# fhgyuanshen/HybridGL

Measured on AMD Instinct MI355X. Metric: images/sec (whole node), higher is better.
Workload: dtype f32 via fp16x3 split MFMA (fp32 accumulate)

## Files before the change

### hybridgl_amd/_lib.py

```python
import ctypes as C
import os

_HERE = os.path.dirname(os.path.abspath(__file__))
LIB_PATH = os.path.join(_HERE, "libhybridgl.so")

c_float_p = C.POINTER(C.c_float)
c_u8_p = C.POINTER(C.c_uint8)
c_i32_p = C.POINTER(C.c_int32)
c_i64_p = C.POINTER(C.c_int64)


class HybridGLError(RuntimeError):
    pass


class HglSentence(C.Structure):
    _fields_ = [("sentence_row", C.c_int), ("noun_phrase_row", C.c_int), ("other_row0", C.c_int), ("n_other", C.c_int),
                ("dirflag", C.c_int), ("relaword", C.c_int), ("has_other_nouns", C.c_int), ("black", C.c_float),
                ("imgattn", C.c_void_p), ("target", C.c_void_p)]


class HglGroupRef(C.Structure):
    _fields_ = [("hybrid", C.c_void_p), ("text", C.c_void_p), ("T", C.c_int), ("boxes", C.c_void_p), ("masks", C.c_void_p),
                ("N", C.c_int), ("H", C.c_int), ("W", C.c_int), ("sentences", C.POINTER(HglSentence)), ("S", C.c_int),
# ... 141 lines not shown
                                  _VP, _VP, _SZ, _VP]),
    "hgl_sam_relpos_tables_workspace_bytes": (_SZ, [_I, _I, _I, _I]),
    "hgl_sam_relpos_tables": (_I, [_VP, _VP, _VP, _I, _I, _I, _I, _I, _I, _VP, _VP, _VP, _VP, _VP, _SZ, _VP]),
    "hgl_sam_dense_pe": (_I, [C.POINTER(HglSamDecoderW), _VP, _VP, _VP]),
    "hgl_sam_decode_workspace_bytes": (_SZ, [C.POINTER(HglSamDecoderW), _I]),
    "hgl_sam_decode_points": (_I, [C.POINTER(HglSamDecoderW), _VP, _VP, _I, _VP, _VP, _VP, _SZ, _VP]),
    "hgl_sam_decode_points_gated": (_I, [C.POINTER(HglSamDecoderW), _VP, _VP, _I, C.c_float, _VP, _VP, _VP, _SZ, _VP]),
    "hgl_sam_decode_multi_workspace_bytes": (_SZ, [C.POINTER(HglSamDecoderW), _I, _I]),
    "hgl_sam_decode_points_multi": (_I, [C.POINTER(HglSamDecoderW), _VP, _VP, _I, _I, _VP, _VP, _VP, _SZ, _VP]),
    "hgl_sam_decode_points_multi_gated": (_I, [C.POINTER(HglSamDecoderW), _VP, _VP, _I, _I, C.c_float, _VP, _VP, _VP, _SZ, _VP]),
    "hgl_sam_decode_prompts": (_I, [C.POINTER(HglSamDecoderW), _VP, _VP, _VP, _I, _VP, _I, _I, _VP, _VP, _VP, _SZ, _VP]),
    "hgl_sam_embed_masks": (_I, [C.POINTER(HglSamDecoderW), _VP, _I, _VP, _VP]),
    "hgl_sam_decoder_fusion": (_I, [_I]),
    "hgl_attention_presplit": (_I, [_I]),
    "hgl_attention_presplit_f32": (_I, [_VP, _I, _I, _I, _I, _I, _VP, _I, C.c_float, _I, _VP, _I, _I, _VP, C.c_size_t, _VP]),
    "hgl_sam_postprocess_workspace_bytes": (_SZ, [_I]),
    "hgl_sam_postprocess": (_I, [_VP, _VP, _I, _I, _I, _I, _I, _I, _I, _I, _F, _F, _F, _F, _VP, _VP, _VP, _VP, _VP,
                                 _VP, _SZ, _VP]),
    "hgl_nms": (_I, [_VP, _VP, _VP, _I, _F, _VP, _VP, _VP]),
    "hgl_nms_segments": (_I, [_VP, _VP, _VP, _VP, _I, _I, _F, _VP, _VP, _VP]),
    "hgl_nms_large_workspace_bytes": (_SZ, [_I]),
    "hgl_nms_large": (_I, [_VP, _VP, _VP, _I, _F, _VP, _VP, _VP, _SZ, _VP]),
    "hgl_box_near_crop_edge": (_I, [_VP, _I, C.POINTER(C.c_int32), C.POINTER(C.c_int32), _F, _VP, _VP]),
    "hgl_remove_small_regions_workspace_bytes": (_SZ, [_I, _I, _I]),
    "hgl_remove_small_regions": (_I, [_VP, _I, _I, _I, _I, _I, _VP, _VP, _VP, _SZ, _VP]),
    "hgl_remove_small_regions_boxes": (_I, [_VP, _I, _I, _I, _I, _I, _VP, _VP, _VP, _VP, _SZ, _VP]),
    "hgl_mask_boxes": (_I, [_VP, _I, _I, _I, _VP, _VP]),
    "hgl_gather_masks": (_I, [_VP, _VP, _VP, _I, _LL, _VP, _VP]),
    "hgl_gen_dir_mask": (_I, [_I, _I, _I, _VP, _VP]),
    "hgl_relation_boxes": (_I, [_VP, _VP, _VP, _VP, _I, _I, _VP, _VP]),
# ... 74 lines not shown
```

### hybridgl_amd/csrc/attention_ps.hip

```cpp
#include "hgl_common.h"
#include "attn_tile.h"
#include <stdlib.h>
#include <mutex>
#include <type_traits>

namespace {

typedef __attribute__((address_space(3))) void lds_void_t;

constexpr int PS_CHUNK = 32;

enum { PS_PLAIN = 0, PS_WIN14 = 1, PS_RELT = 2 };

struct PsArgs {
  const _Float16 *hi, *lo;
  int ld, qcol, kcol, vcol;
  long long sb;
  int B, H, S;
  float* out;
  _Float16 *out_hi, *out_lo;
  int ldo;
  long long sob;
  float scale;
  int mask_kind;
  const uint8_t* keep;
  int keep_b0, keep_n;
  const float *rel_h, *rel_w;
  int kh, kw;
  const _Float16 *tabh_hi, *tabh_lo, *tabw_hi, *tabw_lo;
  int nqb;
  int dbg;
};
#ifdef HGL_DIAG
#define PS_DBG(a) ((a).dbg)
#else
#define PS_DBG(a) 0
#endif

__device__ __forceinline__ void ps_glds16(const void* sbase, unsigned voff, unsigned lds_addr) {
  unsigned keep;
  asm volatile("s_mov_b32 %0, m0\n\ts_mov_b32 m0, %3\n\ts_nop 0\n\tglobal_load_lds_dwordx4 %1, %2\n\ts_mov_b32 m0, %0"
               : "=&s"(keep)
               : "v"(voff), "s"(sbase), "s"(lds_addr)
               : "memory");
// ... 293 lines not shown
      const unsigned krow = min((unsigned)(ci * PS_CHUNK) + v_row[j], (unsigned)(a.S - 1));
      ps_glds16(kv_base, krow * ldb + v_col[j], sbase + (unsigned)(wave + 4 * j) * 1024u);
    }
  };
  const int nchunk = (a.S + PS_CHUNK - 1) / PS_CHUNK;
  if constexpr (MODE == PS_WIN14) {
    for (int i = wave; i < PSP_EBYTES / 1024; i += 4) ps_glds16(etab, (unsigned)(i * 1024 + lane * 16), lds0 + G::E_OFF + (unsigned)i * 1024u);
  }
  const int tr_off = attn_tr_off<VP>(lane, h);
  const int k_off = r * KP + 8 * h;
  int e_off[2];
#pragma unroll
  for (int c = 0; c < 2; ++c) e_off[c] = r * 64 + (((2 * c + h) ^ ((r >> 2) & 3)) * 16);

  const unsigned nunits = (unsigned)(a.B * a.H) * (unsigned)a.nqb;
  for (unsigned L = blockIdx.x; L < nunits; L += gridDim.x) {
  int item, bx;
  {
    const unsigned nqb = (unsigned)a.nqb;
    if ((a.B & 7) == 0) {
      int be, rem;
      attn_xcd_item(L, (unsigned)a.H * nqb, be, rem);
      item = (int)((unsigned)be * (unsigned)a.H + (unsigned)rem / nqb);
      bx = (int)((unsigned)rem % nqb);
    } else {
      item = (int)(L / nqb);
      bx = (int)(L % nqb);
    }
  }
  const int b = item / a.H, hh = item - b * a.H;
  kv_base = (const char*)a.hi + ((long long)b * a.sb * (long long)a.ld + a.kcol + hh * HD) * 2;
  if (L != blockIdx.x) __syncthreads();
  if (!(PS_DBG(a) & 4)) {
  issue_k(0);
  issue_v(0);
// ... 342 lines not shown
            const auto s0 = __builtin_amdgcn_permlane32_swap(x[0], y[0], false, false);
            const auto s1 = __builtin_amdgcn_permlane32_swap(x[1], y[1], false, false);
            return u32x4s{(unsigned)s0[0], (unsigned)s1[0], (unsigned)s0[1], (unsigned)s1[1]};
          };
          const u32x4s vh = pair16(hi0, hi1), vl = pair16(lo0, lo1);
          if (qvalid[qt]) {
            const long long off = orow + d * 32 + 8 * g + 8 * h;
            *(u32x4s*)(a.out_hi + off) = vh;
            *(u32x4s*)(a.out_lo + off) = vl;
          }
        }
      }
  }
  }
  }
}

const unsigned char* psp_etab() {
  static const unsigned char* tab[64] = {nullptr};
  static std::mutex mu;
  std::lock_guard<std::mutex> lk(mu);
  int dev = 0;
  if (hipGetDevice(&dev) != hipSuccess || dev < 0 || dev >= 64) dev = 0;
  if (!tab[dev]) {
    static unsigned short host[PS_EROWS * 32];
    for (int row = 0; row < PS_EROWS; ++row)
      for (int j = 0; j < 32; ++j) {
        const int ih = row / 14, iw = 14 + row % 14;
        const int chunk = j >> 3, phys = chunk ^ ((row >> 2) & 3);
        host[row * 32 + phys * 8 + (j & 7)] = (j == ih || j == iw) ? 0x3c00 : 0;
// ... 51 lines not shown
#ifdef HGL_PS_STAMPS
extern "C" int hgl_debug_ps_stamps(unsigned long long* out, int n, int block, int wave) {
  (void)hipMemcpyFromSymbol(out, HIP_SYMBOL(g_ps_stamps), sizeof(unsigned long long) * (n < 1024 ? n : 1024));
  unsigned long long z[1024] = {0};
  (void)hipMemcpyToSymbol(HIP_SYMBOL(g_ps_stamps), z, sizeof(z));
  int sel[2] = {block, wave};
  (void)hipMemcpyToSymbol(HIP_SYMBOL(g_ps_stamp_sel), sel, sizeof(sel));
  return 0;
}
#endif

extern "C" int hgl_attention_presplit(int on) {
  const int prev = attn_ps_flag();
  if (on >= 0) g_attn_ps = on != 0;
  return prev;
}

HglAttnRoute hgl_attention_route_planes(const HglAttn& d) {
  const int S = d.Sq, hd = d.hd;
  if (!(attn_ps_flag() != 0 && hgl_split_layout() && hgl_split_terms() == 3) || d.Sk != S) return HGL_ATTN_NONE;
  if (!(hd == 80 || hd == 64) || d.mask_kind == HGL_MASK_CAUSAL || d.B <= 0 || d.H <= 0 || S <= 0) return HGL_ATTN_NONE;
  const long long plane_delta = (const char*)d.qkv_lo - (const char*)d.qkv_hi;
  const long long span = (long long)S * d.ld * 2 + (long long)d.ld * 2;
  if (plane_delta < 0 || plane_delta + span >= (1ll << 32)) return HGL_ATTN_NONE;
  static const int clip_kernel = HGL_DIAG_SWITCH("HGL_ATTN_PS_CLIP", 1);
  const int rel_kh = d.rel_h ? d.kh : 0, rel_kw = d.rel_h ? d.kw : 0;
  if (d.tab_h || d.tab_w) {
    const void* t[4];
    return hd == 80 && S == 196 && d.mask_kind == HGL_MASK_NONE && !rel_kh && hgl_attention_rel_tables(d.tab_h, d.tab_w, t)
               ? HGL_ATTN_PS_WIN
// ... 16 lines not shown
  HGL_REQUIRE((d.ld & 7) == 0 && (d.qcol & 7) == 0 && (d.kcol & 7) == 0 && (d.vcol & 7) == 0 && (d.ldo & 3) == 0 && (d.sob & 3) == 0 &&
                  (((uintptr_t)d.qkv_hi | (uintptr_t)d.qkv_lo | (uintptr_t)d.out | (uintptr_t)d.out_hi | (uintptr_t)d.out_lo) & 15) == 0,
              "attention_ps: operands must be 16-byte aligned");
  HGL_REQUIRE(d.mask_kind != HGL_MASK_CLS_KEEP || d.keep, "attention_ps: HGL_MASK_CLS_KEEP needs keep bytes");
  HGL_REQUIRE(d.vcol >= d.kcol, "attention_ps: the V columns must not lie before the K columns (32-bit offsets from the K base)");
  HGL_REQUIRE((d.rel_h == nullptr) == (d.rel_w == nullptr) && (d.tab_h == nullptr) == (d.tab_w == nullptr), "attention_ps: rel-pos operands go in pairs");
  PsArgs a;
  a.hi = (const _Float16*)d.qkv_hi; a.lo = (const _Float16*)d.qkv_lo;
  a.ld = d.ld; a.qcol = d.qcol; a.kcol = d.kcol; a.vcol = d.vcol; a.sb = d.sb;
  a.B = d.B; a.H = d.H; a.S = S;
  a.out = d.out; a.out_hi = (_Float16*)d.out_hi; a.out_lo = (_Float16*)d.out_lo; a.ldo = d.ldo; a.sob = d.sob;
  a.scale = d.scale; a.mask_kind = d.mask_kind; a.keep = d.keep; a.keep_b0 = d.keep_b0; a.keep_n = d.keep_n > 0 ? d.keep_n : d.B;
  a.rel_h = d.rel_h; a.rel_w = d.rel_w; a.kh = d.kh; a.kw = d.kw;
  a.tabh_hi = a.tabh_lo = a.tabw_hi = a.tabw_lo = nullptr;
  a.nqb = 1;
  a.dbg = HGL_DIAG_SWITCH("HGL_ATTN_PS_DBG", 0);
  if (route == HGL_ATTN_PS_WIN) {
    const void* t[4];
    (void)hgl_attention_rel_tables(d.tab_h, d.tab_w, t);
    a.tabh_hi = (const _Float16*)t[0]; a.tabh_lo = (const _Float16*)t[1];
    a.tabw_hi = (const _Float16*)t[2]; a.tabw_lo = (const _Float16*)t[3];
    a.nqb = 2;
  } else if (route != HGL_ATTN_PS_CLIP) {
    a.nqb = (S + 127) / 128;
  }
  HglProfScope prof(HGL_PROF_ATTN, 4.0 * d.B * d.H * (double)S * S * d.hd, 0.0, st);
  switch (route) {
    case HGL_ATTN_PS_WIN: return psp_launch<80, PS_WIN14>(a, st);
    case HGL_ATTN_PS_RELT: return d.hd == 80 ? psp_launch<80, PS_RELT>(a, st) : psp_launch<64, PS_RELT>(a, st);
    case HGL_ATTN_PS_PLAIN: return d.hd == 80 ? psp_launch<80, PS_PLAIN>(a, st) : psp_launch<64, PS_PLAIN>(a, st);
    default: return ps_launch<64, PS_PLAIN, 2>(a, st);
  }
}

extern "C" int hgl_attention_presplit_f32(const float* qkv, int ld, int B, int H, int S, int hd, float* out, int ldo, float scale,
                                          int mask_kind, const uint8_t* keep, int keep_b0, int keep_n, void* scratch,
                                          size_t scratch_bytes, void* stream) {
// ... 5 lines not shown
  hipStream_t st = (hipStream_t)stream;
  uint16_t* hi = (uint16_t*)scratch;
  uint16_t* lo = hi + n;
  HGL_TRY(hgl_launch_split_f16(qkv, 1.0f, hi, lo, (long long)n, st));
  HglAttn d = hgl_attn_packed_planes(hi, lo, B, H, S, hd);
  d.ld = ld, d.scale = scale;
  d.out = out, d.ldo = ldo, d.sob = (long long)S * ldo;
  d.mask_kind = mask_kind, d.keep = keep, d.keep_b0 = keep_b0, d.keep_n = keep_n;
  const int prev = hgl_attention_presplit(1);
  const bool served = hgl_attention_route(d) != HGL_ATTN_NONE;
  const int rc = served ? hgl_launch_attention(d, st) : HGL_OK;
  hgl_attention_presplit(prev);
  HGL_REQUIRE(served, "attention_presplit: shape not served (B %d, H %d, S %d, hd %d, mask %d)", B, H, S, hd, mask_kind);
  return rc;
}
```

### hybridgl_amd/csrc/hgl_common.h

```cpp
#pragma once
#include <hip/hip_runtime.h>
#include <stdint.h>
#include <stddef.h>
#include <math.h>
#include <atomic>
#include <type_traits>
#include "../../include/hybridgl.h"

typedef float f32x16 __attribute__((ext_vector_type(16)));
typedef float f32x4 __attribute__((ext_vector_type(4)));

#ifdef __HIPCC__
static __device__ __attribute__((unused)) unsigned int hgl_tu_split_overflow;
__device__ __forceinline__ void hgl_split_hi_lo(float x, _Float16& hi, _Float16& lo) {
  asm volatile("" : "+v"(x));
  hi = (_Float16)x;
  lo = (_Float16)(x - (float)hi);
}
__device__ __forceinline__ void hgl_split_hi_lo(float x, _Float16& hi, _Float16& lo, float& amax) {
  asm volatile("" : "+v"(x));
  amax = fmaxf(amax, fabsf(x));
  hi = (_Float16)x;
  lo = (_Float16)(x - (float)hi);
}
// ... 171 lines not shown
  int ldq = 0, ldk = 0, ldv = 0;
  long long sqb = 0, skb = 0, svb = 0;
  const void *qkv_hi = nullptr, *qkv_lo = nullptr;
  int ld = 0, qcol = 0, kcol = 0, vcol = 0;
  long long sb = 0;
  float* out = nullptr;
  void *out_hi = nullptr, *out_lo = nullptr;
  int ldo = 0;
  long long sob = 0;
  int mask_kind = HGL_MASK_NONE;
  const uint8_t* keep = nullptr;
  int keep_b0 = 0, keep_n = 0;
  const float *rel_h = nullptr, *rel_w = nullptr;
  int kh = 0, kw = 0;
  const float *tab_h = nullptr, *tab_w = nullptr;
  float* part = nullptr;
  size_t part_bytes = 0;
  int kv_group = 1;
};
inline HglAttn hgl_attn_packed(const float* qkv, int B, int H, int S, int hd) {
  const int D = H * hd;
  HglAttn d;
  d.B = B, d.H = H, d.Sq = S, d.Sk = S, d.hd = hd, d.scale = 1.0f / sqrtf((float)hd);
  d.q = qkv, d.k = qkv + D, d.v = qkv + 2 * D;
  d.ldq = d.ldk = d.ldv = 3 * D;
  d.sqb = d.skb = d.svb = (long long)S * 3 * D;
  d.ldo = D, d.sob = (long long)S * D;
  return d;
}
inline HglAttn hgl_attn_packed_planes(const void* hi, const void* lo, int B, int H, int S, int hd) {
// ... 13 lines not shown
  HGL_ATTN_SMALLK,
  HGL_ATTN_F32,
  HGL_ATTN_PINGPONG,
  HGL_ATTN_REL14,
  HGL_ATTN_DUAL,
  HGL_ATTN_WIDE,
  HGL_ATTN_TILE,
  HGL_ATTN_PS_WIN,
  HGL_ATTN_PS_RELT,
  HGL_ATTN_PS_CLIP,
  HGL_ATTN_PS_PLAIN
};
HglAttnRoute hgl_attention_route(const HglAttn& d);
int hgl_launch_attention(const HglAttn& d, hipStream_t st);
size_t hgl_attention_fewq_part_bytes(int B, int Sk);
bool hgl_attention_rel_tables(const float* tab_h, const float* tab_w, const void* t[4]);
HglAttnRoute hgl_attention_route_planes(const HglAttn& d);
int hgl_launch_attention_planes(const HglAttn& d, HglAttnRoute route, hipStream_t st);

int hgl_launch_im2col_patch(const float* img, int N, int res, int patch, float* cols, hipStream_t st);
int hgl_launch_im2col_patch_split(const float* img, int N, int res, int patch, void* hi, void* lo, hipStream_t st);
int hgl_launch_assemble_lnpre(const float* tok, const float* cls, const float* pos, const float* lw,
                              const float* lb, float* x, int B, int S, int D, hipStream_t st);
int hgl_launch_mask_resize(const uint8_t* masks, int N, int Hm, int Wm, int g, float* pm,
                           uint8_t* keep, hipStream_t st);
int hgl_launch_mix(float* out, const float* a, float ca, const float* b, float cb, const float* pm,
                   int N, int S, int D, hipStream_t st);
int hgl_launch_gather_rows(const float* x, long long row_stride, int rows, int D, float* y,
                           hipStream_t st);
int hgl_launch_add_inplace(float* y, const float* x, long long n, hipStream_t st);
// ... 40 lines not shown
                             float* rel, hipStream_t st);
int hgl_launch_relpos_direct(const float* qkv, int ldq, int B, int heads, int S, int size, int hd,
                             const float* Rh, const float* Rw, float* rel_h, float* rel_w, hipStream_t st);
int hgl_launch_relpos_split(const void* q_hi, const void* q_lo, int ldq, int B, int heads, int S, int size, int hd,
                            const float* Rh, const float* Rw, float* rel_h, float* rel_w, hipStream_t st);
int hgl_launch_im2col3x3(const float* in, int g, int C, float* cols, hipStream_t st);
int hgl_launch_add_rows_bcast(const float* a, long long a_bstride, const float* pe, long long rows_elems,
                              int B, float* out, hipStream_t st);
int hgl_launch_pe(const float* coords01, const float* G, int n, int F, int mode, const float* pos_embed,
                  const float* not_a_point, float* out, hipStream_t st);
int hgl_launch_build_tokens(const float* iou_tok, const float* mask_tok, const float* sparse, int P, int C, int T,
                            float* tokens, hipStream_t st);
int hgl_launch_mask_downscaling(const float* in, int P, int g, const float* c1w, const float* c1b, const float* n1w, const float* n1b,
                                const float* c2w, const float* c2b, const float* n2w, const float* n2b, const float* c3w,
                                const float* c3b, float* out, hipStream_t st);
int hgl_launch_win_maps(int g, int ws, int nw, int nb, int* pad_of, int* tok_of, int* pad_list, int* pad_count, hipStream_t st);
int hgl_launch_fill_rows(float* dst, int ld, const int* rows, const int* nrows, int max_rows, const float* v, int N,
                         hipStream_t st);
int hgl_launch_fill_rows_split(void* hi, void* lo, int ld, const int* rows, const int* nrows, int max_rows, const float* v,
                               int N, hipStream_t st);
int hgl_launch_ln_gelu64(float* x, const float* w, const float* b, long long rows, float eps, void* hi, void* lo,
                         hipStream_t st);
int hgl_launch_ln256_pe_split(float* x, const float* w, const float* b, const float* pe, int pe_rows, long long rows,
                              float eps, int write_f32, void* kh, void* kl, void* ph, void* pl, hipStream_t st);
int hgl_launch_hyper_logits(const float* u2, const float* hyper, int P, int g, int row0, float* low_res, hipStream_t st);
int hgl_launch_pe_labeled(const float* coords01, const int32_t* labels, const float* G, int n, int F, const float* not_a_point,
                          const float* const* point_embed, float* out, hipStream_t st);
int hgl_launch_t2i_fold_q(const float* q1, const float* Wk, float scale, float* Qk, int P, hipStream_t st);
int hgl_t2i_key_ranges(int P, int HW);
size_t hgl_t2i_part_bytes(int P, int HW);
int hgl_launch_t2i_raw_attn(const void* Qh, const void* Ql, const float* bias, const void* Kh, const void* Kl, int P, int HW,
// ... 36 lines not shown
```

### hybridgl_amd/csrc/sam_api.hip

```cpp
#include "hgl_common.h"
#include <stdlib.h>
#include <math.h>

namespace {

struct EncPlan {
  float *img, *cols, *X, *H, *Hw, *QKV, *O, *P, *F, *Th, *Tw, *relh, *relw, *neckA, *neckB, *cols3;
  int *pad_of, *tok_of, *pad_list, *pad_count;
  int n_pad_max;
  int nb;
};

bool carve_enc(HglArena& ar, const HglSamEncoderW* w, int nb, EncPlan& p) {
  const int D = w->embed_dim, S = w->img_size, g = S / w->patch, C = w->out_chans;
  const size_t T = (size_t)nb * g * g;
  size_t Tw_max = T;
  int rl_max = 0, size_max = 0;
  for (int i = 0; i < w->depth; ++i) {
    const int ws = w->blocks[i].window;
    if (ws > 0) {
      const size_t nw = (g + ws - 1) / ws;
      Tw_max = Tw_max > nb * nw * nw * ws * ws ? Tw_max : nb * nw * nw * ws * ws;
    }
    rl_max = rl_max > w->blocks[i].rel_len ? rl_max : w->blocks[i].rel_len;
    size_max = size_max > (ws > 0 ? ws : g) ? size_max : (ws > 0 ? ws : g);
  }
  p.nb = nb;
  p.img = ar.take<float>((size_t)nb * 3 * S * S);
  p.cols = ar.take<float>(T * 3 * w->patch * w->patch);
  p.X = ar.take<float>(T * D);
  p.H = ar.take<float>(T * D);
  p.Hw = ar.take<float>(Tw_max * D);
  p.QKV = ar.take<float>(Tw_max * 3 * D);
  p.O = ar.take<float>(Tw_max * D);
  p.P = ar.take<float>(Tw_max * D);
  p.F = ar.take<float>(T * 4 * D);
  p.Th = ar.take<float>((size_t)w->heads * Tw_max * rl_max);
  p.Tw = ar.take<float>((size_t)w->heads * Tw_max * rl_max);
  p.relh = ar.take<float>((size_t)w->heads * Tw_max * size_max);
  p.relw = ar.take<float>((size_t)w->heads * Tw_max * size_max);
  p.neckA = ar.take<float>(T * C);
  p.neckB = ar.take<float>(T * C);
  p.cols3 = ar.take<float>(T * C * 9);
  p.pad_of = ar.take<int>(T);
  p.tok_of = ar.take<int>(T);
  p.n_pad_max = (int)(Tw_max - T);
  p.pad_list = ar.take<int>(Tw_max - T + 1);
  p.pad_count = ar.take<int>(1);
  return ar.ok();
}

bool valid_enc(const HglSamEncoderW* w) {
  return w && w->embed_dim > 0 && w->depth > 0 && w->heads > 0 && w->img_size > 0 && w->patch > 0 &&
         w->out_chans > 0 && w->img_size % w->patch == 0 && w->embed_dim % w->heads == 0 &&
         (w->embed_dim & 3) == 0 && w->patch_w && w->patch_b && w->pos_embed && w->blocks && w->neck0_w &&
         w->neck1_w && w->neck1_b && w->neck2_w && w->neck3_w && w->neck3_b;
}

enum EncAttn {
  ENC_ATTN_PS_WIN,
  ENC_ATTN_PS_GLOBAL,
  ENC_ATTN_WIN14,
  ENC_ATTN_TABLES
};

struct EncBlockRoute {
  int D, g, heads, hd;
  int T1, T;
  int ws, size, nw;
  int B1, B;
  int S, M1, M;
  int L;
  bool x3;
  EncAttn attn;
  bool gather;
  bool planes;
};

struct EncPlanes {
  uint16_t *Ah, *Al;
  uint16_t *Hh, *Hl;
  uint16_t *Fh, *Fl;
  uint16_t *Qh, *Ql;
  EncPlanes(const EncPlan& p, const EncBlockRoute& r)
      : Ah((uint16_t*)p.Hw), Al(Ah + (size_t)r.M * r.D), Hh((uint16_t*)p.H), Hl(Hh + (size_t)r.T * r.D), Fh((uint16_t*)p.F),
        Fl(Fh + (size_t)r.T * 4 * r.D), Qh((uint16_t*)p.QKV), Ql(Qh + (size_t)r.M * 3 * r.D) {}
};

HglAttn enc_attn(const HglSamBlockW& b, const EncPlan& p, const EncBlockRoute& r, EncAttn kind) {
  const EncPlanes s(p, r);
  const bool planes = kind == ENC_ATTN_PS_WIN || kind == ENC_ATTN_PS_GLOBAL;
  HglAttn d = planes ? hgl_attn_packed_planes(s.Qh, s.Ql, r.B, r.heads, r.S, r.hd) : hgl_attn_packed(p.QKV, r.B, r.heads, r.S, r.hd);
  d.out = r.x3 ? nullptr : p.O, d.out_hi = s.Ah, d.out_lo = s.Al;
  if (kind == ENC_ATTN_PS_WIN || kind == ENC_ATTN_WIN14) d.tab_h = b.rel_pos_h, d.tab_w = b.rel_pos_w;
  else d.rel_h = p.relh, d.rel_w = p.relw, d.kh = d.kw = r.size;
  return d;
}

int enc_block_route(const HglSamEncoderW* w, const HglSamBlockW& b, const EncPlan& p, EncBlockRoute& r) {
  const int nb = p.nb;
  r.D = w->embed_dim, r.g = w->img_size / w->patch, r.heads = w->heads, r.hd = r.D / r.heads;
  r.T1 = r.g * r.g, r.T = nb * r.T1;
  r.ws = b.window, r.size = r.ws > 0 ? r.ws : r.g, r.nw = r.ws > 0 ? (r.g + r.ws - 1) / r.ws : 1;
  r.B1 = r.nw * r.nw, r.B = nb * r.B1;
  r.S = r.size * r.size, r.M1 = r.B1 * r.S, r.M = r.B * r.S;
  r.L = b.rel_len;
  HGL_REQUIRE(r.L == 2 * r.size - 1, "sam_encode: rel_pos length %d does not match attention size %d", r.L, r.size);
  const int D = r.D;
  r.x3 = hgl_use_x3(b.qkv_w, D) && hgl_use_x3(b.proj_w, D) && hgl_use_x3(b.lin1_w, D) && hgl_use_x3(b.lin2_w, 4 * D) &&
         (D % 256) == 0;
  static const int padskip = HGL_DIAG_SWITCH("HGL_SAM_PADSKIP", 1);
  r.gather = r.x3 && r.ws > 0 && r.M > r.T && padskip;
  static const int ps_glob_on = HGL_DIAG_SWITCH("HGL_ATTN_PS_GLOBAL", 1);
  const auto serves = [&](EncAttn kind, HglAttnRoute family) { return hgl_attention_route(enc_attn(b, p, r, kind)) == family; };
  r.attn = ENC_ATTN_TABLES;
  if (r.x3 && r.ws == 14 && serves(ENC_ATTN_PS_WIN, HGL_ATTN_PS_WIN)) r.attn = ENC_ATTN_PS_WIN;
  else if (r.x3 && r.ws == 0 && r.size == 64 && ps_glob_on && serves(ENC_ATTN_PS_GLOBAL, HGL_ATTN_PS_RELT)) r.attn = ENC_ATTN_PS_GLOBAL;
  else if (r.x3 && r.ws == 14 && serves(ENC_ATTN_WIN14, HGL_ATTN_WIN14)) r.attn = ENC_ATTN_WIN14;
  r.planes = r.attn == ENC_ATTN_PS_WIN || r.attn == ENC_ATTN_PS_GLOBAL;
  return HGL_OK;
}

int enc_relpos_tables(const float* qkv, const void* q_hi, const void* q_lo, int ldq, int B, int heads, int S, int size, int hd,
                      const float* Rh, const float* Rw, float* rel_h, float* rel_w, float* Th, float* Tw, hipStream_t st) {
  if (q_hi || q_lo) return hgl_launch_relpos_split(q_hi, q_lo, ldq, B, heads, S, size, hd, Rh, Rw, rel_h, rel_w, st);
  if ((hd == 80 || hd == 64) && (size & 1) == 0 && size <= 64)
    return hgl_launch_relpos_direct(qkv, ldq, B, heads, S, size, hd, Rh, Rw, rel_h, rel_w, st);
// ... 428 lines not shown
    uint16_t* ch = (uint16_t*)p.cols;
    uint16_t* cl = ch + (size_t)T * kd;
    HGL_TRY(hgl_launch_im2col_patch_split(p.img, nb, S, w->patch, ch, cl, st));
    HglGemm embed = hgl_gemm_planes(ch, cl, w->patch_w, w->patch_b, p.X, T, D, kd, HGL_ACT_NONE, w->pos_embed);
    embed.rmod = nb > 1 ? T1 : 0;
    HGL_TRY(hgl_launch_gemm(embed, st));
  } else {
    HGL_TRY(hgl_launch_im2col_patch(p.img, nb, S, w->patch, p.cols, st));
    HglGemm embed = hgl_gemm_linear(p.cols, w->patch_w, w->patch_b, p.X, T1, D, kd, HGL_ACT_NONE, w->pos_embed);
    embed.batch = nb, embed.sA = (long long)T1 * kd, embed.sC = (long long)T1 * D;
    HGL_TRY(hgl_launch_gemm(embed, st));
  }
  for (int i = 0; i < w->depth; ++i) {
    const int ws = w->blocks[i].window;
    if (ws > 0) {
      HGL_TRY(hgl_launch_win_maps(g, ws, (g + ws - 1) / ws, nb, p.pad_of, p.tok_of, p.pad_list, p.pad_count, st));
      break;
    }
  }
  for (int i = 0; i < w->depth; ++i) HGL_TRY(enc_block(w, w->blocks[i], p, st));
  const bool neck_x3 = hgl_use_x3(w->neck0_w, D) && hgl_use_x3(w->neck2_w, C * 9);
  if (neck_x3) {
    uint16_t* xh = (uint16_t*)p.H;
    uint16_t* xl = xh + (size_t)T * D;
    HGL_TRY(hgl_launch_split_f16(p.X, 1.0f, xh, xl, (long long)T * D, st));
    HGL_TRY(hgl_launch_gemm(hgl_gemm_planes(xh, xl, w->neck0_w, nullptr, p.neckA, T, C, D), st));
  } else {
    HGL_TRY(hgl_launch_gemm(hgl_gemm_linear(p.X, w->neck0_w, nullptr, p.neckA, T, C, D), st));
  }
  HGL_TRY(hgl_launch_layernorm(p.neckA, w->neck1_w, w->neck1_b, p.neckB, T, C, 1e-6f, st));
  for (int i = 0; i < nb; ++i)
// ... 53 lines not shown
  return hgl_launch_pe(grid_coords01, w->pe_gauss, w->grid * w->grid, w->C / 2, 0, nullptr, nullptr, dense_pe,
                       (hipStream_t)stream);
}

size_t hgl_sam_decode_workspace_bytes(const HglSamDecoderW* w, int P) {
  if (!valid_dec(w) || P <= 0) return 0;
  HglArena ar(nullptr, 0);
  DecPlan p;
  carve_dec(ar, w, P, p);
  return ar.off;
}

int hgl_sam_decoder_fusion(int mask) {
  const int old = dec_fusion_mask();
  if (mask >= 0) g_dec_fusion = mask;
  return old;
}

__global__ void iou_gate_kernel(const float* __restrict__ iou, int P, float gate, uint8_t* __restrict__ skip) {
  const int p = blockIdx.x * blockDim.x + threadIdx.x;
  if (p >= P) return;
  skip[p] = (iou[3 * p] > gate || iou[3 * p + 1] > gate || iou[3 * p + 2] > gate) ? 0 : 1;
}

static int decode_impl(const HglSamDecoderW* w, const float* emb, const float* points01, const float* coords01,
                       const int32_t* labels, int n_sparse, const float* dense, int first_mask, int P, float* low_res,
                       float* iou_pred, void* workspace, size_t workspace_bytes, void* stream, bool gated = false,
                       float iou_gate = 0.f, int n_img = 1) {
  const HglSplitTermsScope three_terms(3);
  HGL_TRY(hgl_require_device());
// ... 177 lines not shown
```

### hybridgl_amd/csrc/sam_glue.hip

```cpp
#include "hgl_common.h"
#include "post_geom.h"
#include <math.h>

typedef float f32x2 __attribute__((ext_vector_type(2)));
typedef _Float16 f16x4g __attribute__((ext_vector_type(4)));
typedef unsigned u32x4g __attribute__((ext_vector_type(4)));

namespace {

inline unsigned grid1(long long n, int block = 256) { return (unsigned)((n + block - 1) / block); }

__global__ __launch_bounds__(256) void sam_preprocess_kernel(const uint8_t* __restrict__ img, int h, int w,
                                                             int S, float* __restrict__ out) {
  const long long i = blockIdx.x * 256ll + threadIdx.x;
  if (i >= 3ll * S * S) return;
  const int x = (int)(i % S), y = (int)((i / S) % S), c = (int)(i / ((long long)S * S));
  const float mean[3] = {123.675f, 116.28f, 103.53f};
  const float stdv[3] = {58.395f, 57.12f, 57.375f};
  float v = 0.f;
  if (y < h && x < w) v = ((float)img[((long long)y * w + x) * 3 + c] - mean[c]) / stdv[c];
  out[i] = v;
}

__global__ __launch_bounds__(256) void pil_resample_kernel(const uint8_t* __restrict__ in, uint8_t* __restrict__ out,
// ... 259 lines not shown
      const int k0 = h ? sp : 0, k1 = h ? size : sp;
      const float* src = Gw + qc + size - 1;
      for (int k = k0; k < k1; k += 2) {
        f32x2 o;
        o[0] = src[-k];
        o[1] = src[-k - 1];
        *(f32x2*)(out + k) = o;
      }
    }
    }
  }
}

__global__ __launch_bounds__(256) void win_maps_kernel(int g, int ws, int nw, int nb, int* __restrict__ pad_of,
                                                       int* __restrict__ tok_of, int* __restrict__ pad_list,
                                                       int* __restrict__ pad_count) {
  const int Tw = nw * nw * ws * ws;
  const int gidx = blockIdx.x * 256 + threadIdx.x;
  if (gidx >= nb * Tw) return;
  const int img = gidx / Tw, idx = gidx - img * Tw;
  const int w = idx / (ws * ws), p = idx - w * ws * ws;
  const int wy = w / nw, wx = w - wy * nw, py = p / ws, px = p - py * ws;
  const int y = wy * ws + py, x = wx * ws + px;
  if (y < g && x < g) {
    const int rh = min(ws, g - wy * ws), rw = min(ws, g - wx * ws);
    const int r = img * g * g + wy * ws * g + rh * (wx * ws) + py * rw + px;
    pad_of[r] = gidx;
    tok_of[r] = img * g * g + y * g + x;
  } else {
    pad_list[atomicAdd(pad_count, 1)] = gidx;
  }
}

__global__ __launch_bounds__(256) void fill_rows_kernel(float* __restrict__ dst, int ld, const int* __restrict__ rows,
                                                        const int* __restrict__ nrows, const float* __restrict__ v, int N4) {
  const int i = blockIdx.y;
  if (i >= *nrows) return;
  f32x4* d = (f32x4*)(dst + (long long)rows[i] * ld);
  for (int c = blockIdx.x * 256 + threadIdx.x; c < N4; c += gridDim.x * 256) d[c] = ((const f32x4*)v)[c];
}
// ... 624 lines not shown
  const dim3 gridm((unsigned)((S + qpw - 1) / qpw), (unsigned)(B * heads), 1);
  const size_t ldsm = (size_t)2 * NT * 32 * (hd + 8) * sizeof(_Float16) + (size_t)4 * 32 * (NT * 32 + 1) * sizeof(float);
#define HGL_RPS_LAUNCH(HD_, NT_)                                                                                         \
  do {                                                                                                                 \
    HGL_RESERVE_LDS((relpos_mfma_kernel<HD_, NT_, true>), ldsm, "relpos_split");                                        \
    hipLaunchKernelGGL((relpos_mfma_kernel<HD_, NT_, true>), gridm, dim3(256), ldsm, st, (const float*)nullptr, ldq, heads, S, size, Rh, \
                       Rw, rel_h, rel_w, (const _Float16*)q_hi, (const _Float16*)q_lo);                                \
  } while (0)
  if (hd == 80 && NT == 1) HGL_RPS_LAUNCH(80, 1);
  else if (hd == 80) HGL_RPS_LAUNCH(80, 4);
  else if (NT == 1) HGL_RPS_LAUNCH(64, 1);
  else HGL_RPS_LAUNCH(64, 4);
#undef HGL_RPS_LAUNCH
  return hgl_check_launch("relpos_split");
}
int hgl_launch_win_maps(int g, int ws, int nw, int nb, int* pad_of, int* tok_of, int* pad_list, int* pad_count, hipStream_t st) {
  if (hipMemsetAsync(pad_count, 0, sizeof(int), st) != hipSuccess) {
    hgl_set_error("win_maps: memset failed");
    return HGL_ELAUNCH;
  }
  hipLaunchKernelGGL(win_maps_kernel, dim3(grid1((long long)nb * nw * nw * ws * ws)), dim3(256), 0, st, g, ws, nw, nb, pad_of,
                     tok_of, pad_list, pad_count);
  return hgl_check_launch("win_maps");
}
int hgl_launch_fill_rows(float* dst, int ld, const int* rows, const int* nrows, int max_rows, const float* v, int N,
                         hipStream_t st) {
  HGL_REQUIRE((N & 3) == 0 && max_rows > 0, "fill_rows: bad arguments");
  hipLaunchKernelGGL(fill_rows_kernel, dim3(4, (unsigned)max_rows), dim3(256), 0, st, dst, ld, rows, nrows, v, N / 4);
  return hgl_check_launch("fill_rows");
}
int hgl_launch_fill_rows_split(void* hi, void* lo, int ld, const int* rows, const int* nrows, int max_rows, const float* v,
                               int N, hipStream_t st) {
  HGL_REQUIRE((N & 3) == 0 && (ld & 3) == 0 && max_rows > 0 && hi && lo, "fill_rows_split: bad arguments");
  hipLaunchKernelGGL(fill_rows_split_kernel, dim3(4, (unsigned)max_rows), dim3(256), 0, st, (_Float16*)hi,
                     hgl_split_terms() == 1 ? nullptr : (_Float16*)lo, ld, rows,
                     nrows, v, N / 4);
  return hgl_check_launch("fill_rows_split");
// ... 130 lines not shown
```

### hybridgl_amd/ops.py

```python
import ctypes as C
from itertools import repeat

import torch

from . import _lib
from ._lib import check

ACT = {"none": 0, "quickgelu": 1, "gelu": 2, "relu": 3}
MASK = {"none": 0, "causal": 1, "cls_keep": 2}
DIRFLAG = {"none": 0, "left": 1, "right": 2, "middle": 3}
RELAWORD = {"none": 0, "left": 1, "right": 2, "up": 3, "down": 4, "big": 5, "small": 6, "within": 7}


def _stream():
    return torch.cuda.current_stream().cuda_stream


def _dev(t, dtype, name):
    if not isinstance(t, torch.Tensor):
        raise TypeError(f"{name}: expected a torch.Tensor")
    if not t.is_cuda:
        raise _lib.HybridGLError(f"{name}: tensor must live on the GPU (no CPU path exists)")
    if t.dtype != dtype:
        raise TypeError(f"{name}: expected dtype {dtype}, got {t.dtype}")
# ... 214 lines not shown
    lib = _lib.load()
    B, S, D3 = qkv.shape
    Dm = D3 // 3
    hd = Dm // heads
    if scale is None:
        scale = hd ** -0.5
    out = torch.empty((B, S, Dm), dtype=torch.float32, device=qkv.device)
    scratch = torch.empty(B * S * D3, dtype=torch.float32, device=qkv.device)
    kp = None
    if keep is not None:
        kp, keep = _u8(keep, "keep")
    check(lib.hgl_attention_presplit_f32(_dev(qkv, torch.float32, "qkv"), D3, B, heads, S, hd, _dev(out, torch.float32, "out"), Dm,
                                         float(scale), MASK[mask], kp, keep_b0, keep_n, scratch.data_ptr(), scratch.numel() * 4,
                                         _stream()), "hgl_attention_presplit_f32")
    return out


def sam_relpos_tables(q, rel_pos_h, rel_pos_w, B, heads, size, rel_h=None, rel_w=None):
    lib = _lib.load()
    S = size * size
    hd = rel_pos_h.shape[1]
    planes = isinstance(q, (tuple, list))
    q0 = q[0] if planes else q
    assert q0.shape[0] == B * S and tuple(rel_pos_h.shape) == tuple(rel_pos_w.shape) == (2 * size - 1, hd)
    if rel_h is None:
        rel_h = torch.empty((B * heads, S, size), dtype=torch.float32, device=q0.device)
    if rel_w is None:
        rel_w = torch.empty((B * heads, S, size), dtype=torch.float32, device=q0.device)
    assert tuple(rel_h.shape) == tuple(rel_w.shape) == (B * heads, S, size)
    need = lib.hgl_sam_relpos_tables_workspace_bytes(B, heads, S, size)
# ... 814 lines not shown
```

### include/hybridgl.h

```cpp
#ifndef HYBRIDGL_H
#define HYBRIDGL_H

#include <stddef.h>
#include <stdint.h>

#ifdef __cplusplus
extern "C" {
#endif

#define HGL_OK 0
#define HGL_EINVAL (-1)
#define HGL_ENODEVICE (-2)
#define HGL_EWORKSPACE (-3)
#define HGL_ELAUNCH (-4)

#define HGL_ABI_VERSION 7

#define HGL_ACT_NONE 0
#define HGL_ACT_QUICKGELU 1
#define HGL_ACT_GELU 2
#define HGL_ACT_RELU 3

#define HGL_FUSION_G2L 0
#define HGL_FUSION_L2G 1
// ... 281 lines not shown
                                float* low_res, float* iou_pred, void* workspace, size_t workspace_bytes, void* stream);
int hgl_sam_decode_points_multi_gated(const HglSamDecoderW* w, const float* emb, const float* points01, int n_img, int ppi,
                                      float iou_gate, float* low_res, float* iou_pred, void* workspace, size_t workspace_bytes,
                                      void* stream);
int hgl_sam_decode_prompts(const HglSamDecoderW* w, const float* emb, const float* coords01, const int32_t* labels, int n_sparse,
                           const float* dense, int first_mask, int P, float* low_res, float* iou_pred, void* workspace,
                           size_t workspace_bytes, void* stream);
int hgl_sam_embed_masks(const HglSamDecoderW* w, const float* mask_input, int P, float* dense, void* stream);

int hgl_sam_decoder_fusion(int mask);

int hgl_attention_presplit(int on);
int hgl_attention_presplit_f32(const float* qkv, int ld, int B, int H, int S, int hd, float* out, int ldo, float scale,
                               int mask_kind, const uint8_t* keep, int keep_b0, int keep_n, void* scratch,
                               size_t scratch_bytes, void* stream);

size_t hgl_sam_postprocess_workspace_bytes(int K);
int hgl_sam_postprocess(const float* low_res, const float* iou_pred, int K, int hl, int wl, int img_size,
                        int in_h, int in_w, int H, int W, float mask_threshold, float stability_offset,
                        float pred_iou_thresh, float stability_thresh, uint8_t* masks, int32_t* boxes_xyxy,
                        float* stability, uint8_t* keep, float* full_logits, void* workspace,
                        size_t workspace_bytes, void* stream);

int hgl_nms(const int32_t* boxes_xyxy, const float* scores, const uint8_t* keep, int K, float iou_threshold,
            int32_t* out_idx, int32_t* out_n, void* stream);

int hgl_nms_segments(const int32_t* boxes_xyxy, const float* scores, const uint8_t* keep, const int32_t* offsets, int n_seg,
                     int max_len, float iou_threshold, int32_t* out_idx, int32_t* out_n, void* stream);

size_t hgl_remove_small_regions_workspace_bytes(int N, int H, int W);
// ... 81 lines not shown
```

Measured before the change: 34.68.

## Skip fully padded query blocks in SAM windowed attention via live-unit list

Measured after the change: 34.85 (median of 6 runs). About the same (+0.5%).

```diff
diff --git a/hybridgl_amd/_lib.py b/hybridgl_amd/_lib.py
--- a/hybridgl_amd/_lib.py
+++ b/hybridgl_amd/_lib.py
@@ -179,6 +179,8 @@
     "hgl_sam_decoder_fusion": (_I, [_I]),
     "hgl_attention_presplit": (_I, [_I]),
     "hgl_attention_presplit_f32": (_I, [_VP, _I, _I, _I, _I, _I, _VP, _I, C.c_float, _I, _VP, _I, _I, _VP, C.c_size_t, _VP]),
+    "hgl_attention_presplit_win_f32": (_I, [_VP, _I, _I, _I, _VP, _I, C.c_float, _VP, _VP, _VP, _VP, C.c_size_t, _VP]),
+    "hgl_sam_window_skip": (_I, [_I]),
     "hgl_sam_postprocess_workspace_bytes": (_SZ, [_I]),
     "hgl_sam_postprocess": (_I, [_VP, _VP, _I, _I, _I, _I, _I, _I, _I, _I, _F, _F, _F, _F, _VP, _VP, _VP, _VP, _VP,
                                  _VP, _SZ, _VP]),
diff --git a/hybridgl_amd/csrc/attention_ps.hip b/hybridgl_amd/csrc/attention_ps.hip
--- a/hybridgl_amd/csrc/attention_ps.hip
+++ b/hybridgl_amd/csrc/attention_ps.hip
@@ -28,6 +28,7 @@
   const float *rel_h, *rel_w;
   int kh, kw;
   const _Float16 *tabh_hi, *tabh_lo, *tabw_hi, *tabw_lo;
+  const int* units;
   int nqb;
   int dbg;
 };
@@ -351,11 +352,28 @@
   for (int c = 0; c < 2; ++c) e_off[c] = r * 64 + (((2 * c + h) ^ ((r >> 2) & 3)) * 16);
 
   const unsigned nunits = (unsigned)(a.B * a.H) * (unsigned)a.nqb;
-  for (unsigned L = blockIdx.x; L < nunits; L += gridDim.x) {
+  const bool live_walk = MODE == PS_WIN14 && a.units != nullptr;
+  const unsigned nwalk = live_walk ? (unsigned)a.units[0] : nunits;
+  int* const aheadL = (int*)keepL;
+  unsigned step = 0;
+  for (unsigned L = blockIdx.x; L < nwalk; L += gridDim.x, ++step) {
   int item, bx;
   {
     const unsigned nqb = (unsigned)a.nqb;
-    if ((a.B & 7) == 0) {
+    if (live_walk) {
+      if ((step & 63u) == 0) {
+        if (step) __syncthreads();
+        if (t < 64) {
+          const unsigned La = L + (unsigned)t * gridDim.x;
+          aheadL[t] = La < nwalk ? a.units[1u + La] : -1;
+        }
+        __syncthreads();
+      }
+      const int u = __builtin_amdgcn_readfirstlane(aheadL[step & 63u]);
+      if (u < 0) continue;
+      item = (int)((unsigned)u / nqb);
+      bx = (int)((unsigned)u % nqb);
+    } else if ((a.B & 7) == 0) {
       int be, rem;
       attn_xcd_item(L, (unsigned)a.H * nqb, be, rem);
       item = (int)((unsigned)be * (unsigned)a.H + (unsigned)rem / nqb);
@@ -728,6 +746,43 @@
   }
   }
   }
+  if (live_walk) asm volatile("s_waitcnt vmcnt(0)" ::: "memory");
+}
+
+constexpr int PSP_WIN_NQB = 2, PSP_WIN_ROWS = 128;
+__global__ __launch_bounds__(256) void psp_live_units_kernel(const int* __restrict__ q_live, int B, int H, int* __restrict__ units) {
+  __shared__ int scan[256];
+  __shared__ int len[8];
+  const int t = threadIdx.x;
+  int maxlen = 0;
+  for (int c = 0; c < 8; ++c) {
+    const int ne = c < B ? (B - c + 7) / 8 : 0;
+    int base = 0;
+    for (int k0 = 0; k0 < ne; k0 += 256) {
+      const int k = k0 + t;
+      int nl = 0;
+      if (k < ne) nl = min(PSP_WIN_NQB, max(0, (q_live[c + 8 * k] + PSP_WIN_ROWS - 1) / PSP_WIN_ROWS));
+      const int n = H * nl;
+      scan[t] = n;
+      __syncthreads();
+      for (int d = 1; d < 256; d <<= 1) {
+        const int v = t >= d ? scan[t - d] : 0;
+        __syncthreads();
+        scan[t] += v;
+        __syncthreads();
+      }
+      const int start = base + scan[t] - n;
+      base += scan[255];
+      __syncthreads();
+      for (int s = 0; s < n; ++s) units[1 + (start + s) * 8 + c] = ((c + 8 * k) * H + s / nl) * PSP_WIN_NQB + s % nl;
+    }
+    if (t == 0) len[c] = base;
+    maxlen = max(maxlen, base);
+  }
+  __syncthreads();
+  for (int c = 0; c < 8; ++c)
+    for (int i = len[c] + t; i < maxlen; i += 256) units[1 + i * 8 + c] = -1;
+  if (t == 0) units[0] = 8 * maxlen;
 }
 
 const unsigned char* psp_etab() {
@@ -809,6 +864,13 @@
   const int prev = attn_ps_flag();
   if (on >= 0) g_attn_ps = on != 0;
   return prev;
+}
+
+size_t hgl_attention_live_units_ints(int B, int H) { return 1 + (size_t)8 * ((B + 7) / 8) * H * PSP_WIN_NQB; }
+int hgl_launch_attention_live_units(const int* q_live, int B, int H, int* units, hipStream_t st) {
+  HGL_REQUIRE(q_live && units && B > 0 && H > 0, "attention_live_units: bad arguments");
+  hipLaunchKernelGGL(psp_live_units_kernel, dim3(1), dim3(256), 0, st, q_live, B, H, units);
+  return hgl_check_launch("attention_live_units");
 }
 
 HglAttnRoute hgl_attention_route_planes(const HglAttn& d) {
@@ -855,13 +917,15 @@
   a.rel_h = d.rel_h; a.rel_w = d.rel_w; a.kh = d.kh; a.kw = d.kw;
   a.tabh_hi = a.tabh_lo = a.tabw_hi = a.tabw_lo = nullptr;
   a.nqb = 1;
+  HGL_REQUIRE((d.q_live == nullptr) == (d.live_units == nullptr), "attention_ps: q_live and live_units go together");
+  a.units = route == HGL_ATTN_PS_WIN ? d.live_units : nullptr;
   a.dbg = HGL_DIAG_SWITCH("HGL_ATTN_PS_DBG", 0);
   if (route == HGL_ATTN_PS_WIN) {
     const void* t[4];
     (void)hgl_attention_rel_tables(d.tab_h, d.tab_w, t);
     a.tabh_hi = (const _Float16*)t[0]; a.tabh_lo = (const _Float16*)t[1];
     a.tabw_hi = (const _Float16*)t[2]; a.tabw_lo = (const _Float16*)t[3];
-    a.nqb = 2;
+    a.nqb = PSP_WIN_NQB;
   } else if (route != HGL_ATTN_PS_CLIP) {
     a.nqb = (S + 127) / 128;
   }
@@ -897,3 +961,34 @@
   HGL_REQUIRE(served, "attention_presplit: shape not served (B %d, H %d, S %d, hd %d, mask %d)", B, H, S, hd, mask_kind);
   return rc;
 }
+
+extern "C" int hgl_attention_presplit_win_f32(const float* qkv, int ld, int B, int H, float* out, int ldo, float scale, const float* tab_h,
+                                              const float* tab_w, const int* q_live, void* scratch, size_t scratch_bytes,
+                                              void* stream) {
+  HGL_TRY(hgl_require_device());
+  const int S = 196, hd = 80;
+  HGL_REQUIRE(qkv && out && scratch && tab_h && tab_w && B > 0 && H > 0 && ld >= 3 * H * hd && (ld & 7) == 0 && ldo >= H * hd,
+              "attention_presplit_win: bad arguments");
+  const size_t n = (size_t)B * S * ld, need = (n + (q_live ? hgl_attention_live_units_ints(B, H) : 0)) * 4;
+  HGL_REQUIRE(scratch_bytes >= need, "attention_presplit_win: scratch too small (%zu bytes for %zu)", scratch_bytes, need);
+  HGL_REQUIRE(hgl_split_layout() && hgl_split_terms() == 3, "attention_presplit_win: f16x3 mode only");
+  hipStream_t st = (hipStream_t)stream;
+  uint16_t* hi = (uint16_t*)scratch;
+  uint16_t* lo = hi + n;
+  HGL_TRY(hgl_launch_split_f16(qkv, 1.0f, hi, lo, (long long)n, st));
+  HglAttn d = hgl_attn_packed_planes(hi, lo, B, H, S, hd);
+  d.ld = ld, d.scale = scale;
+  d.out = out, d.ldo = ldo, d.sob = (long long)S * ldo;
+  d.tab_h = tab_h, d.tab_w = tab_w;
+  if (q_live) {
+    int* units = (int*)(lo + n);
+    HGL_TRY(hgl_launch_attention_live_units(q_live, B, H, units, st));
+    d.q_live = q_live, d.live_units = units;
+  }
+  const int prev = hgl_attention_presplit(1);
+  const bool served = hgl_attention_route(d) == HGL_ATTN_PS_WIN;
+  const int rc = served ? hgl_launch_attention(d, st) : HGL_OK;
+  hgl_attention_presplit(prev);
+  HGL_REQUIRE(served, "attention_presplit_win: not served (B %d, H %d; are the tables registered at scale 2^0?)", B, H);
+  return rc;
+}
diff --git a/hybridgl_amd/csrc/hgl_common.h b/hybridgl_amd/csrc/hgl_common.h
--- a/hybridgl_amd/csrc/hgl_common.h
+++ b/hybridgl_amd/csrc/hgl_common.h
@@ -209,6 +209,8 @@
   const float *rel_h = nullptr, *rel_w = nullptr;
   int kh = 0, kw = 0;
   const float *tab_h = nullptr, *tab_w = nullptr;
+  const int* q_live = nullptr;
+  const int* live_units = nullptr;
   float* part = nullptr;
   size_t part_bytes = 0;
   int kv_group = 1;
@@ -252,6 +254,8 @@
 HglAttnRoute hgl_attention_route(const HglAttn& d);
 int hgl_launch_attention(const HglAttn& d, hipStream_t st);
 size_t hgl_attention_fewq_part_bytes(int B, int Sk);
+size_t hgl_attention_live_units_ints(int B, int H);
+int hgl_launch_attention_live_units(const int* q_live, int B, int H, int* units, hipStream_t st);
 bool hgl_attention_rel_tables(const float* tab_h, const float* tab_w, const void* t[4]);
 HglAttnRoute hgl_attention_route_planes(const HglAttn& d);
 int hgl_launch_attention_planes(const HglAttn& d, HglAttnRoute route, hipStream_t st);
@@ -322,7 +326,8 @@
 int hgl_launch_mask_downscaling(const float* in, int P, int g, const float* c1w, const float* c1b, const float* n1w, const float* n1b,
                                 const float* c2w, const float* c2b, const float* n2w, const float* n2b, const float* c3w,
                                 const float* c3b, float* out, hipStream_t st);
-int hgl_launch_win_maps(int g, int ws, int nw, int nb, int* pad_of, int* tok_of, int* pad_list, int* pad_count, hipStream_t st);
+int hgl_launch_win_maps(int g, int ws, int nw, int nb, int* pad_of, int* tok_of, int* pad_list, int* pad_count, int* q_live,
+                        hipStream_t st);
 int hgl_launch_fill_rows(float* dst, int ld, const int* rows, const int* nrows, int max_rows, const float* v, int N,
                          hipStream_t st);
 int hgl_launch_fill_rows_split(void* hi, void* lo, int ld, const int* rows, const int* nrows, int max_rows, const float* v,
diff --git a/hybridgl_amd/csrc/sam_api.hip b/hybridgl_amd/csrc/sam_api.hip
--- a/hybridgl_amd/csrc/sam_api.hip
+++ b/hybridgl_amd/csrc/sam_api.hip
@@ -7,6 +7,7 @@
 struct EncPlan {
   float *img, *cols, *X, *H, *Hw, *QKV, *O, *P, *F, *Th, *Tw, *relh, *relw, *neckA, *neckB, *cols3;
   int *pad_of, *tok_of, *pad_list, *pad_count;
+  int *q_live, *live_units;
   int n_pad_max;
   int nb;
 };
@@ -14,13 +15,14 @@
 bool carve_enc(HglArena& ar, const HglSamEncoderW* w, int nb, EncPlan& p) {
   const int D = w->embed_dim, S = w->img_size, g = S / w->patch, C = w->out_chans;
   const size_t T = (size_t)nb * g * g;
-  size_t Tw_max = T;
+  size_t Tw_max = T, nwin_max = 1;
   int rl_max = 0, size_max = 0;
   for (int i = 0; i < w->depth; ++i) {
     const int ws = w->blocks[i].window;
     if (ws > 0) {
       const size_t nw = (g + ws - 1) / ws;
       Tw_max = Tw_max > nb * nw * nw * ws * ws ? Tw_max : nb * nw * nw * ws * ws;
+      nwin_max = nwin_max > nb * nw * nw ? nwin_max : nb * nw * nw;
     }
     rl_max = rl_max > w->blocks[i].rel_len ? rl_max : w->blocks[i].rel_len;
     size_max = size_max > (ws > 0 ? ws : g) ? size_max : (ws > 0 ? ws : g);
@@ -47,6 +49,8 @@
   p.n_pad_max = (int)(Tw_max - T);
   p.pad_list = ar.take<int>(Tw_max - T + 1);
   p.pad_count = ar.take<int>(1);
+  p.q_live = ar.take<int>(nwin_max);
+  p.live_units = ar.take<int>(hgl_attention_live_units_ints((int)nwin_max, w->heads));
   return ar.ok();
 }
 
@@ -74,6 +78,7 @@
   bool x3;
   EncAttn attn;
   bool gather;
+  bool live;
   bool planes;
 };
 
@@ -94,7 +99,14 @@
   d.out = r.x3 ? nullptr : p.O, d.out_hi = s.Ah, d.out_lo = s.Al;
   if (kind == ENC_ATTN_PS_WIN || kind == ENC_ATTN_WIN14) d.tab_h = b.rel_pos_h, d.tab_w = b.rel_pos_w;
   else d.rel_h = p.relh, d.rel_w = p.relw, d.kh = d.kw = r.size;
+  if (kind == ENC_ATTN_PS_WIN && r.live) d.q_live = p.q_live, d.live_units = p.live_units;
   return d;
+}
+
+int g_win_skip = -1;
+int win_skip_flag() {
+  if (g_win_skip < 0) g_win_skip = HGL_DIAG_SWITCH("HGL_SAM_WIN_SKIP", 1) != 0;
+  return g_win_skip;
 }
 
 int enc_block_route(const HglSamEncoderW* w, const HglSamBlockW& b, const EncPlan& p, EncBlockRoute& r) {
@@ -111,6 +123,7 @@
          (D % 256) == 0;
   static const int padskip = HGL_DIAG_SWITCH("HGL_SAM_PADSKIP", 1);
   r.gather = r.x3 && r.ws > 0 && r.M > r.T && padskip;
+  r.live = r.gather && win_skip_flag();
   static const int ps_glob_on = HGL_DIAG_SWITCH("HGL_ATTN_PS_GLOBAL", 1);
   const auto serves = [&](EncAttn kind, HglAttnRoute family) { return hgl_attention_route(enc_attn(b, p, r, kind)) == family; };
   r.attn = ENC_ATTN_TABLES;
@@ -569,7 +582,9 @@
   for (int i = 0; i < w->depth; ++i) {
     const int ws = w->blocks[i].window;
     if (ws > 0) {
-      HGL_TRY(hgl_launch_win_maps(g, ws, (g + ws - 1) / ws, nb, p.pad_of, p.tok_of, p.pad_list, p.pad_count, st));
+      const int nw = (g + ws - 1) / ws;
+      HGL_TRY(hgl_launch_win_maps(g, ws, nw, nb, p.pad_of, p.tok_of, p.pad_list, p.pad_count, p.q_live, st));
+      if (g % ws != 0 && win_skip_flag()) HGL_TRY(hgl_launch_attention_live_units(p.q_live, nb * nw * nw, w->heads, p.live_units, st));
       break;
     }
   }
@@ -653,6 +668,12 @@
 int hgl_sam_decoder_fusion(int mask) {
   const int old = dec_fusion_mask();
   if (mask >= 0) g_dec_fusion = mask;
+  return old;
+}
+
+int hgl_sam_window_skip(int on) {
+  const int old = win_skip_flag();
+  if (on >= 0) g_win_skip = on != 0;
   return old;
 }
 
diff --git a/hybridgl_amd/csrc/sam_glue.hip b/hybridgl_amd/csrc/sam_glue.hip
--- a/hybridgl_amd/csrc/sam_glue.hip
+++ b/hybridgl_amd/csrc/sam_glue.hip
@@ -297,7 +297,7 @@
 
 __global__ __launch_bounds__(256) void win_maps_kernel(int g, int ws, int nw, int nb, int* __restrict__ pad_of,
                                                        int* __restrict__ tok_of, int* __restrict__ pad_list,
-                                                       int* __restrict__ pad_count) {
+                                                       int* __restrict__ pad_count, int* __restrict__ q_live) {
   const int Tw = nw * nw * ws * ws;
   const int gidx = blockIdx.x * 256 + threadIdx.x;
   if (gidx >= nb * Tw) return;
@@ -305,8 +305,9 @@
   const int w = idx / (ws * ws), p = idx - w * ws * ws;
   const int wy = w / nw, wx = w - wy * nw, py = p / ws, px = p - py * ws;
   const int y = wy * ws + py, x = wx * ws + px;
+  const int rh = min(ws, g - wy * ws), rw = min(ws, g - wx * ws);
+  if (p == 0) q_live[img * nw * nw + w] = (rh - 1) * ws + rw;
   if (y < g && x < g) {
-    const int rh = min(ws, g - wy * ws), rw = min(ws, g - wx * ws);
     const int r = img * g * g + wy * ws * g + rh * (wx * ws) + py * rw + px;
     pad_of[r] = gidx;
     tok_of[r] = img * g * g + y * g + x;
@@ -961,13 +962,14 @@
 #undef HGL_RPS_LAUNCH
   return hgl_check_launch("relpos_split");
 }
-int hgl_launch_win_maps(int g, int ws, int nw, int nb, int* pad_of, int* tok_of, int* pad_list, int* pad_count, hipStream_t st) {
+int hgl_launch_win_maps(int g, int ws, int nw, int nb, int* pad_of, int* tok_of, int* pad_list, int* pad_count, int* q_live,
+                        hipStream_t st) {
   if (hipMemsetAsync(pad_count, 0, sizeof(int), st) != hipSuccess) {
     hgl_set_error("win_maps: memset failed");
     return HGL_ELAUNCH;
   }
   hipLaunchKernelGGL(win_maps_kernel, dim3(grid1((long long)nb * nw * nw * ws * ws)), dim3(256), 0, st, g, ws, nw, nb, pad_of,
-                     tok_of, pad_list, pad_count);
+                     tok_of, pad_list, pad_count, q_live);
   return hgl_check_launch("win_maps");
 }
 int hgl_launch_fill_rows(float* dst, int ld, const int* rows, const int* nrows, int max_rows, const float* v, int N,
diff --git a/hybridgl_amd/ops.py b/hybridgl_amd/ops.py
--- a/hybridgl_amd/ops.py
+++ b/hybridgl_amd/ops.py
@@ -252,6 +252,30 @@
                                          float(scale), MASK[mask], kp, keep_b0, keep_n, scratch.data_ptr(), scratch.numel() * 4,
                                          _stream()), "hgl_attention_presplit_f32")
     return out
+
+
+def attention_presplit_win(qkv, heads, tab_h, tab_w, q_live=None, out=None, scale=None):
+    lib = _lib.load()
+    B, S, D3 = qkv.shape
+    Dm = D3 // 3
+    hd = Dm // heads
+    if S != 196 or hd != 80:
+        raise ValueError("attention_presplit_win: 196 tokens at head dim 80 only")
+    if scale is None:
+        scale = hd ** -0.5
+    if out is None:
+        out = torch.empty((B, S, Dm), dtype=torch.float32, device=qkv.device)
+    units = 1 + 8 * ((B + 7) // 8) * heads * 2 if q_live is not None else 0
+    planes = torch.empty(B * S * D3 + units, dtype=torch.float32, device=qkv.device)
+    check(lib.hgl_attention_presplit_win_f32(_dev(qkv, torch.float32, "qkv"), D3, B, heads, _dev(out, torch.float32, "out"), Dm,
+                                             float(scale), _dev(tab_h, torch.float32, "tab_h"), _dev(tab_w, torch.float32, "tab_w"),
+                                             _dev(q_live, torch.int32, "q_live") if q_live is not None else None,
+                                             planes.data_ptr(), planes.numel() * 4, _stream()), "hgl_attention_presplit_win_f32")
+    return out
+
+
+def sam_window_skip(on=-1):
+    return _lib.load().hgl_sam_window_skip(int(on))
 
 
 def sam_relpos_tables(q, rel_pos_h, rel_pos_w, B, heads, size, rel_h=None, rel_w=None):
diff --git a/include/hybridgl.h b/include/hybridgl.h
--- a/include/hybridgl.h
+++ b/include/hybridgl.h
@@ -319,6 +319,9 @@
 int hgl_attention_presplit_f32(const float* qkv, int ld, int B, int H, int S, int hd, float* out, int ldo, float scale,
                                int mask_kind, const uint8_t* keep, int keep_b0, int keep_n, void* scratch,
                                size_t scratch_bytes, void* stream);
+int hgl_attention_presplit_win_f32(const float* qkv, int ld, int B, int H, float* out, int ldo, float scale, const float* tab_h,
+                                   const float* tab_w, const int* q_live, void* scratch, size_t scratch_bytes, void* stream);
+int hgl_sam_window_skip(int on);
 
 size_t hgl_sam_postprocess_workspace_bytes(int K);
 int hgl_sam_postprocess(const float* low_res, const float* iou_pred, int K, int hl, int wl, int img_size,
```
